# cdglissov/recurrent-flows-msc

Hardware: AMD Instinct MI355X
Metric: frames/sec, RFN SM-MNIST 64x64 train step (fwd+bwd+Adam) (higher is better)
Workload: dtype f32 (forward convolutions fp32-grade: fused scaled-fp16 split f16x3s / three-piece bf16x6 split; gradient convolutions bf16x3 split MFMA; fp32 accumulate everywhere); 1 GPU; RFN SM-MNIST 64x64 canonical (K=10 L=5 Hd=256 h=200 z=56), global_batch=32, seq_len=20, train step; global_batch=32, seq_len=20, parallelism=dp1

## Files before the change

### recurrent-flows-msc_amd/csrc/dgrad_small.hip

```cpp
#include "conv_common.h"
#include <type_traits>

typedef __bf16 bf16x8 __attribute__((ext_vector_type(8)));
typedef __bf16 bf16x4 __attribute__((ext_vector_type(4)));
typedef __bf16 bf16x2 __attribute__((ext_vector_type(2)));

struct DgradSmallParams {
    const float* in;
    long in_ns;
    const unsigned char* wpk;
    float* out1;
    float* out2;
    long out1_ns, out2_ns;
    int Cin, Cout, cout_split, acc1, acc2, CoutP;
    int N, H;
    int CP4;
    int vec;
};

#define DS_MFMA(acc, a, b) acc = __builtin_amdgcn_mfma_f32_32x32x16_bf16(a, b, acc, 0, 0, 0)

template <int CPI>
__device__ __forceinline__ void ds_store_bf16(unsigned char* dst, const __bf16 (&v)[CPI]) {
    if constexpr (CPI == 8) {
        *reinterpret_cast<bf16x8*>(dst) = bf16x8{v[0], v[1], v[2], v[3], v[4], v[5], v[6], v[7]};
    } else if constexpr (CPI == 4) {
        *reinterpret_cast<bf16x4*>(dst) = bf16x4{v[0], v[1], v[2], v[3]};
    } else if constexpr (CPI == 2) {
        *reinterpret_cast<bf16x2*>(dst) = bf16x2{v[0], v[1]};
    } else {
        *reinterpret_cast<__bf16*>(dst) = v[0];
    }
}

template <int W, int MTW, int TPX, int RS>
struct DgradSmallCfg {
    static constexpr int PG = 4 / RS;
    static constexpr int MTT = MTW * RS;
    static constexpr int RPT = 32 / W;
    static constexpr int R = TPX * RPT;
    static constexpr int BPIX = PG * TPX * 32;
    static constexpr bool BAND = BPIX < W * W;
    static constexpr int FPB = BAND ? 1 : BPIX / (W * W);
    static constexpr int PF = BPIX / FPB;
    static constexpr int BR = PF / W;
    static constexpr int IPOSF = (BR + 2) * W, IPOS = FPB * IPOSF;
    static constexpr int IMG_BYTES = 2 * 2 * IPOS * 16;
    static constexpr int WFR = 3 * 2 * MTT;
    static constexpr int WGT_BYTES = WFR * 1024;
    static constexpr int CPI = BPIX / 64;
    static constexpr int NQ = BPIX / 4;
    static constexpr int NLD = CPI + (BAND ? 1 : 0);
    static constexpr int NFI = R + 2 - (RPT - 1);
    static constexpr int ESTR = 36;
    static constexpr int EPI_BYTES = PG * MTT * 32 * ESTR * 4;
    static constexpr int LOOP_BYTES = 2 * IMG_BYTES + 2 * WGT_BYTES;
    static constexpr int LDS_BYTES = LOOP_BYTES > EPI_BYTES ? LOOP_BYTES : EPI_BYTES;
    static_assert(RS == 1 || RS == 2, "row groups");
    static_assert(CPI == 1 || CPI == 2 || CPI == 4 || CPI == 8, "body item shape");
    static_assert(!BAND || W == 32, "bands (halo rows to load) only at W = 32: 2 rows x 16 channels x 8 quads = 256 items");
    static_assert(PF % (TPX * 32) == 0, "a wave's tiles lie in one frame");
    static_assert(LDS_BYTES <= 160 * 1024, "LDS budget");
};

template <int W, int MTW, int TPX, int RS>
__global__ __launch_bounds__(256) void dgrad_small_kernel(const DgradSmallParams p) {
    using C = DgradSmallCfg<W, MTW, TPX, RS>;
    constexpr int PG = C::PG, MTT = C::MTT, RPT = C::RPT, BPIX = C::BPIX, FPB = C::FPB, PF = C::PF, BR = C::BR;
    constexpr int IPOSF = C::IPOSF, IPOS = C::IPOS, IMG_BYTES = C::IMG_BYTES, WFR = C::WFR, WGT_BYTES = C::WGT_BYTES;
    constexpr int CPI = C::CPI, NQ = C::NQ, NLD = C::NLD, NFI = C::NFI, ESTR = C::ESTR;
    constexpr bool BAND = C::BAND;
    constexpr int NJ = (WFR + 3) / 4;
    constexpr unsigned MASKED = 0xFFFFFF00u;
    (void)BPIX; (void)PG;
    extern __shared__ __attribute__((aligned(16))) unsigned char lds[];
    const int tid = threadIdx.x, lane = tid & 63;
    const int wave = __builtin_amdgcn_readfirstlane(tid >> 6);
    const int pg = wave / RS, rs = wave - pg * RS;
    const int l31 = lane & 31, kk = lane >> 5;
    const int HW = p.H * W;
    int n0, rb;
    if (BAND) {
        const int bands = p.H / BR;
        n0 = blockIdx.x / bands;
        rb = (blockIdx.x - n0 * bands) * BR;
    } else {
        n0 = blockIdx.x * FPB;
        rb = 0;
    }
    const int nchunks = p.Cin >> 4;
    const auto rs_in = __builtin_amdgcn_make_buffer_rsrc(const_cast<float*>(p.in), 0,
                                                         (unsigned)((long)p.N * p.in_ns * 4), 0x00020000);

    unsigned b_off, h_off = MASKED;
    int b_dst, h_dst = 0;
    {
        const int cg = tid / NQ, pq = tid - cg * NQ;
        const int f = (pq * 4) / PF, pin = pq * 4 - f * PF;
        const int cl = cg * CPI;
        const bool ok = n0 + f < p.N;
        b_off = ok ? (unsigned)((long)(n0 + f) * p.in_ns * 4) + (unsigned)((cl * HW + rb * W + pin) * 4) : MASKED;
        b_dst = ((cl >> 3) * IPOS + f * IPOSF + W + pin) * 16 + (cl & 7) * 2;
        if (BAND) {
            const int ch = tid >> 4, hr = (tid >> 3) & 1, q = tid & 7;
            const int gy = hr ? rb + BR : rb - 1;
            h_off = (gy >= 0 && gy < p.H) ? (unsigned)((long)n0 * p.in_ns * 4) + (unsigned)((ch * HW + gy * W + 4 * q) * 4)
                                          : MASKED;
            h_dst = ((ch >> 3) * IPOS + (hr ? (BR + 1) * W : 0) + 4 * q) * 16 + (ch & 7) * 2;
        }
    }
    typedef unsigned u32x4_ __attribute__((ext_vector_type(4)));
    auto img_load1 = [&](f32x4 (&raw)[NLD], const int c, const int j) {
        const unsigned base = j < CPI ? b_off : h_off;
        const unsigned off = base == MASKED ? MASKED : base + (unsigned)((c * 16 + (j < CPI ? j : 0)) * HW * 4);
        const u32x4_ v = __builtin_amdgcn_raw_buffer_load_b128(rs_in, off, 0, 0);
        raw[j] = __builtin_bit_cast(f32x4, v);
    };
    auto img_store1 = [&](const f32x4 (&raw)[NLD], const int buf, const int e) {
        unsigned char* img = lds + buf * IMG_BYTES + e * 16;
        __bf16 hi[CPI], lo[CPI];
#pragma unroll
        for (int j = 0; j < CPI; ++j) {
            const float v = raw[j][e];
            hi[j] = (__bf16)v;
            lo[j] = (__bf16)(v - (float)hi[j]);
        }
        ds_store_bf16<CPI>(img + b_dst, hi);
        ds_store_bf16<CPI>(img + b_dst + 2 * IPOS * 16, lo);
        if (BAND) {
            const float v = raw[NLD - 1][e];
            const __bf16 h = (__bf16)v;
            *reinterpret_cast<__bf16*>(img + h_dst) = h;
            *reinterpret_cast<__bf16*>(img + h_dst + 2 * IPOS * 16) = (__bf16)(v - (float)h);
        }
    };
    unsigned w_off[NJ];
#pragma unroll
    for (int j = 0; j < NJ; ++j) {
        const int f = min(wave + 4 * j, WFR - 1);
        const int tp = f / MTT, mt = f - tp * MTT;
        const int dy = tp >> 1, pl = tp & 1;
        const int row = mt * 32 + l31;
        int dx = (row >= p.CP4) + (row >= 2 * p.CP4);
        int co = row - dx * p.CP4;
        if (co >= p.Cout) {
            dx = 0;
            co = p.Cout;
        }
        w_off[j] = (unsigned)((((dy * 3 + dx) * 2 + pl) * 2 + kk) * p.CoutP + co) * 16u;
    }
    const unsigned w_cstride = 36u * (unsigned)p.CoutP * 16u;
    auto wgt_dma = [&](const int c, const int buf) {
        unsigned char* dst0 = lds + 2 * IMG_BYTES + buf * WGT_BYTES;
        const unsigned char* src0 = p.wpk + (size_t)c * w_cstride;
#pragma unroll
        for (int j = 0; j < NJ; ++j) {
            const int f = min(wave + 4 * j, WFR - 1);
            __builtin_amdgcn_global_load_lds((const __attribute__((address_space(1))) void*)(src0 + w_off[j]),
                                             (__attribute__((address_space(3))) void*)(dst0 + f * 1024), 16, 0, 0);
        }
    };
    {
        f32x4* z4 = reinterpret_cast<f32x4*>(lds);
        for (int i = tid; i < 2 * IMG_BYTES / 16; i += 256) z4[i] = f32x4{0.f, 0.f, 0.f, 0.f};
        __syncthreads();
    }

    f32x16 acc[TPX][MTW];
#pragma unroll
    for (int t = 0; t < TPX; ++t)
#pragma unroll
        for (int m = 0; m < MTW; ++m)
#pragma unroll
            for (int r = 0; r < 16; ++r) acc[t][m][r] = 0.f;

    const int wp0 = pg * TPX * 32;
    const int wf = wp0 / PF;
    const int pos0 = wf * IPOSF + (wp0 - wf * PF) + l31;

    f32x4 rawA[NLD], rawB[NLD];
    wgt_dma(0, 0);
#pragma unroll
    for (int j = 0; j < NLD; ++j) img_load1(rawA, 0, j);
#pragma unroll
    for (int j = 0; j < NLD; ++j) img_load1(rawB, 1, j);
#pragma unroll
    for (int e = 0; e < 4; ++e) img_store1(rawA, 0, e);
    asm volatile("s_waitcnt vmcnt(0) lgkmcnt(0)" ::: "memory");
    __syncthreads();

    auto chunk = [&](auto st_, auto ld_, const int c, f32x4 (&rawC)[NLD], f32x4 (&rawN)[NLD]) {
        constexpr bool st = decltype(st_)::value, ld = decltype(ld_)::value;
        const int buf = c & 1;
        const bf16x8* img = reinterpret_cast<const bf16x8*>(lds + buf * IMG_BYTES) + kk * IPOS + pos0;
        const bf16x8* wl = reinterpret_cast<const bf16x8*>(lds + 2 * IMG_BYTES + buf * WGT_BYTES) + rs * MTW * 64 + lane;
        bf16x8 A[3][MTW][2];
#pragma unroll
        for (int dy = 0; dy < 3; ++dy)
#pragma unroll
            for (int m = 0; m < MTW; ++m)
#pragma unroll
                for (int pl = 0; pl < 2; ++pl) A[dy][m][pl] = wl[((dy * 2 + pl) * MTT + m) * 64];
        bf16x8 B[2][2];
        B[0][0] = img[0];
        B[0][1] = img[2 * IPOS];
#pragma unroll
        for (int fi = 0; fi < NFI; ++fi) {
            const int cur = fi & 1;
            if (fi + 1 < NFI) {
                B[cur ^ 1][0] = img[(fi + 1) * W];
                B[cur ^ 1][1] = img[2 * IPOS + (fi + 1) * W];
            }
            __builtin_amdgcn_sched_barrier(0);
#pragma unroll
            for (int combo = 0; combo < 3; ++combo) {
#pragma unroll
                for (int dy = 0; dy < 3; ++dy) {
                    const int ro = (fi - 1) - (dy - 1);
                    if (ro >= 0 && ro <= (TPX - 1) * RPT && ro % RPT == 0) {
#pragma unroll
                        for (int m = 0; m < MTW; ++m) {
                            if (combo == 0) DS_MFMA(acc[ro / RPT][m], A[dy][m][1], B[cur][0]);
                            if (combo == 1) DS_MFMA(acc[ro / RPT][m], A[dy][m][0], B[cur][1]);
                            if (combo == 2) DS_MFMA(acc[ro / RPT][m], A[dy][m][0], B[cur][0]);
                        }
                    }
                }
            }
            constexpr int SS = NFI / 3 > 0 ? NFI / 3 : 1;
#pragma unroll
            for (int k = 0; k < 4; ++k)
                if (st && (k * SS) / 4 == fi) img_store1(rawC, buf ^ 1, k);
            if (st && fi == SS) {
                __builtin_amdgcn_sched_barrier(0);
                wgt_dma(c + 1, buf ^ 1);
                __builtin_amdgcn_sched_barrier(0);
            }
#pragma unroll
            for (int k = 0; k < NLD; ++k)
                if (ld && SS + (k * SS) / NLD == fi) img_load1(rawN, c + 2, k);
            __builtin_amdgcn_sched_barrier(0);
        }
        if (ld) asm volatile("s_waitcnt vmcnt(%0)" ::"n"(NLD) : "memory");
        else asm volatile("s_waitcnt vmcnt(0)" ::: "memory");
        asm volatile("s_waitcnt lgkmcnt(0)" ::: "memory");
        __builtin_amdgcn_s_barrier();
    };
    {
        using T_ = std::integral_constant<bool, true>;
        using F_ = std::integral_constant<bool, false>;
        int c = 0;
        for (; c + 3 < nchunks; c += 2) {
            chunk(T_{}, T_{}, c, rawB, rawA);
            chunk(T_{}, T_{}, c + 1, rawA, rawB);
        }
        chunk(T_{}, F_{}, c, rawB, rawA);
        chunk(F_{}, F_{}, c + 1, rawA, rawB);
    }

    float* E = reinterpret_cast<float*>(lds) + pg * (MTT * 32 * ESTR);
#pragma unroll
    for (int t = 0; t < TPX; ++t) {
        if (t > 0) __syncthreads();
#pragma unroll
        for (int m = 0; m < MTW; ++m)
#pragma unroll
            for (int r = 0; r < 16; ++r)
                E[((rs * MTW + m) * 32 + (r & 3) + 8 * (r >> 2) + 4 * kk) * ESTR + l31] = acc[t][m][r];
        __syncthreads();
        const int wp = wp0 + t * 32;
        const int n = n0 + wf;
        if (n < p.N) {
            const int pix0 = rb * W + (wp - wf * PF);
            for (int idx = rs * 64 + lane; idx < p.Cout * 8; idx += RS * 64) {
                const int co = idx >> 3, q = idx & 7;
                const int x0 = (4 * q) & (W - 1);
                const bool hasL = x0 != 0, hasR = x0 + 4 != W;
                const float* e0 = E + co * ESTR + 4 * q;
                const float* e1 = e0 + p.CP4 * ESTR;
                const float* e2 = e1 + p.CP4 * ESTR;
                const f32x4 a = *reinterpret_cast<const f32x4*>(e0);
                const f32x4 b = *reinterpret_cast<const f32x4*>(e1);
                const f32x4 cc = *reinterpret_cast<const f32x4*>(e2);
                float aL = e0[hasL ? -1 : 0], cR = e2[hasR ? 4 : 0];
                aL = hasL ? aL : 0.f;
                cR = hasR ? cR : 0.f;
                f32x4 o;
                o[0] = aL + b[0] + cc[1];
                o[1] = a[0] + b[1] + cc[2];
                o[2] = a[1] + b[2] + cc[3];
                o[3] = a[2] + b[3] + cR;
                const bool first = co < p.cout_split;
                float* dst = first ? p.out1 + n * p.out1_ns + (long)co * HW + pix0 + 4 * q
                                   : p.out2 + n * p.out2_ns + (long)(co - p.cout_split) * HW + pix0 + 4 * q;
                const bool accm = first ? p.acc1 : p.acc2;
                if (p.vec) {
                    f32x4* d4 = reinterpret_cast<f32x4*>(dst);
                    if (accm) o += *d4;
                    *d4 = o;
                } else {
#pragma unroll
                    for (int e = 0; e < 4; ++e) dst[e] = accm ? o[e] + dst[e] : o[e];
                }
            }
        }
    }
}

template <int W, int MTW, int TPX, int RS>
static int launch_dgrad_small(const DgradSmallParams& p, hipStream_t st) {
    using C = DgradSmallCfg<W, MTW, TPX, RS>;
    constexpr size_t lds = C::LDS_BYTES;
    auto* k = dgrad_small_kernel<W, MTW, TPX, RS>;
    if (lds > 65536) (void)hipFuncSetAttribute((const void*)k, hipFuncAttributeMaxDynamicSharedMemorySize, (int)lds);
    const int blocks = C::BAND ? p.N * (p.H / C::BR) : (p.N + C::FPB - 1) / C::FPB;
    hipLaunchKernelGGL(k, dim3(blocks), dim3(256), lds, st, p);
    return 0;
}

extern "C" int rfn_dgrad_small_supported(int N, int Cin, int Cout, int H, int W) {
    if (N <= 0 || Cin <= 0 || (Cin & 31) || Cout <= 0 || H != W) return 0;
    if ((long)N * Cin * H * W * 4 >= 0xFFFFFF00L) return 0;
    if (W == 32 || W == 16) return Cout <= 64;
    if (W == 8) return Cout <= 96;
    return 0;
}

extern "C" int rfn_conv3x3_smallcout_bf16x3(const float* in, long in_ns, int Cin, const float* wpk, float* out1,
                                            long out1_ns, float* out2, long out2_ns, int Cout, int cout_split, int acc1,
                                            int acc2, int N, int H, int W, rfn_stream_t stream) {
    RFN_CHECK_ARG(in && wpk && out1 && N >= 0, -1);
    RFN_CHECK_ARG(rfn_dgrad_small_supported(N > 0 ? N : 1, Cin, Cout, H, W), -2);
    RFN_CHECK_ARG(cout_split > 0 && cout_split <= Cout && (cout_split == Cout || out2), -3);
    RFN_CHECK_ARG(((uintptr_t)wpk & 15) == 0 && ((uintptr_t)in & 15) == 0 && (in_ns & 3) == 0, -4);
    RFN_CHECK_ARG((long)N * in_ns * 4 < 0xFFFFFF00L && in_ns >= (long)Cin * H * W, -5);
    if (N == 0) return 0;
    DgradSmallParams p;
    p.in = in; p.in_ns = in_ns; p.wpk = reinterpret_cast<const unsigned char*>(wpk);
    p.out1 = out1; p.out2 = out2; p.out1_ns = out1_ns; p.out2_ns = out2_ns;
    p.Cin = Cin; p.Cout = Cout; p.cout_split = cout_split; p.acc1 = acc1; p.acc2 = acc2;
    p.CoutP = ((Cout + 255) / 256) * 256;
    p.N = N; p.H = H;
    p.CP4 = (Cout + 3) & ~3;
    p.vec = ((uintptr_t)out1 & 15) == 0 && (out1_ns & 3) == 0 &&
            (cout_split == Cout || (((uintptr_t)out2 & 15) == 0 && (out2_ns & 3) == 0));
    hipStream_t st = (hipStream_t)stream;
    const int MTR = (3 * p.CP4 + 31) / 32;
    if (W == 32) {
        if (MTR <= 2) launch_dgrad_small<32, 2, 4, 1>(p, st);
        else if (MTR <= 4) launch_dgrad_small<32, 2, 4, 2>(p, st);
        else launch_dgrad_small<32, 3, 4, 2>(p, st);
    } else if (W == 16) {
        if (MTR <= 2) launch_dgrad_small<16, 2, 2, 1>(p, st);
        else if (MTR <= 4) launch_dgrad_small<16, 4, 2, 1>(p, st);
        else launch_dgrad_small<16, 3, 4, 2>(p, st);
    } else {
        if (MTR <= 4) launch_dgrad_small<8, 4, 1, 1>(p, st);
        else if (MTR <= 7 && N >= 512) launch_dgrad_small<8, 7, 1, 1>(p, st);
        else if (MTR <= 8) launch_dgrad_small<8, 4, 1, 2>(p, st);
        else launch_dgrad_small<8, 5, 1, 2>(p, st);
    }
    RFN_LAUNCH_CHECK();
    return 0;
}
```

Before: 12510 frames/s.

## Interleave split-store, weight DMA and MFMA with scheduled groups in dgrad_small chunk loop

Adds a new chunk body for the small dgrad kernel. It issues MFMAs step by step over (dy, tile) and double-buffers the weight fragments in registers. The bf16 hi/lo image split and its LDS writes are spread across those steps. sched_group_barrier enforces an MFMA/DS/VMEM interleave, and the weight DMA is emitted through inline asm with an explicit m0. The aim is to hide LDS traffic, global loads and split arithmetic behind the MFMA pipe. It applies to all configurations except W16/MTW3/TPX4/RS2, and the hand-written asm and strict schedule could raise register pressure or stall.

After: 12540 frames/s, median of 6. About the same (+0.3%).

```diff
diff --git a/recurrent-flows-msc_amd/csrc/dgrad_small.hip b/recurrent-flows-msc_amd/csrc/dgrad_small.hip
--- a/recurrent-flows-msc_amd/csrc/dgrad_small.hip
+++ b/recurrent-flows-msc_amd/csrc/dgrad_small.hip
@@ -56,6 +56,7 @@
     static constexpr int EPI_BYTES = PG * MTT * 32 * ESTR * 4;
     static constexpr int LOOP_BYTES = 2 * IMG_BYTES + 2 * WGT_BYTES;
     static constexpr int LDS_BYTES = LOOP_BYTES > EPI_BYTES ? LOOP_BYTES : EPI_BYTES;
+    static constexpr bool IL = !(W == 16 && MTW == 3 && TPX == 4 && RS == 2);
     static_assert(RS == 1 || RS == 2, "row groups");
     static_assert(CPI == 1 || CPI == 2 || CPI == 4 || CPI == 8, "body item shape");
     static_assert(!BAND || W == 32, "bands (halo rows to load) only at W = 32: 2 rows x 16 channels x 8 quads = 256 items");
@@ -134,6 +135,31 @@
             *reinterpret_cast<__bf16*>(img + h_dst + 2 * IPOS * 16) = (__bf16)(v - (float)h);
         }
     };
+    struct SplitPx {
+        __bf16 hi[CPI], lo[CPI], hh, hl;
+    };
+    auto img_split = [&](const f32x4 (&raw)[NLD], const int e, const int j0, const int j1, SplitPx& sp) {
+#pragma unroll
+        for (int j = j0; j < j1 && j < CPI; ++j) {
+            const float v = raw[j][e];
+            sp.hi[j] = (__bf16)v;
+            sp.lo[j] = (__bf16)(v - (float)sp.hi[j]);
+        }
+        if (BAND && j1 == NLD) {
+            const float v = raw[NLD - 1][e];
+            sp.hh = (__bf16)v;
+            sp.hl = (__bf16)(v - (float)sp.hh);
+        }
+    };
+    auto img_write = [&](const int buf, const int e, const SplitPx& sp) {
+        unsigned char* img = lds + buf * IMG_BYTES + e * 16;
+        ds_store_bf16<CPI>(img + b_dst, sp.hi);
+        ds_store_bf16<CPI>(img + b_dst + 2 * IPOS * 16, sp.lo);
+        if (BAND) {
+            *reinterpret_cast<__bf16*>(img + h_dst) = sp.hh;
+            *reinterpret_cast<__bf16*>(img + h_dst + 2 * IPOS * 16) = sp.hl;
+        }
+    };
     unsigned w_off[NJ];
 #pragma unroll
     for (int j = 0; j < NJ; ++j) {
@@ -160,6 +186,18 @@
                                              (__attribute__((address_space(3))) void*)(dst0 + f * 1024), 16, 0, 0);
         }
     };
+    auto wgt_dma_asm = [&](const int c, const int buf) {
+        const unsigned dst0 = (unsigned)(size_t)(__attribute__((address_space(3))) unsigned char*)(lds + 2 * IMG_BYTES) +
+                              (unsigned)(buf * WGT_BYTES);
+        const unsigned char* src0 = p.wpk + (size_t)c * w_cstride;
+#pragma unroll
+        for (int j = 0; j < NJ; ++j) {
+            const int f = min(wave + 4 * j, WFR - 1);
+            const unsigned m0v = __builtin_amdgcn_readfirstlane(dst0 + (unsigned)f * 1024u);
+            asm volatile("s_mov_b32 m0, %1\n\ts_nop 0\n\tglobal_load_lds_dwordx4 %0, off"
+                         :: "v"(src0 + w_off[j]), "s"(m0v) : "memory");
+        }
+    };
     {
         f32x4* z4 = reinterpret_cast<f32x4*>(lds);
         for (int i = tid; i < 2 * IMG_BYTES / 16; i += 256) z4[i] = f32x4{0.f, 0.f, 0.f, 0.f};
@@ -189,7 +227,83 @@
     asm volatile("s_waitcnt vmcnt(0) lgkmcnt(0)" ::: "memory");
     __syncthreads();
 
-    auto chunk = [&](auto st_, auto ld_, const int c, f32x4 (&rawC)[NLD], f32x4 (&rawN)[NLD]) {
+    auto chunk_il = [&](auto st_, auto ld_, const int c, f32x4 (&rawC)[NLD], f32x4 (&rawN)[NLD]) {
+        constexpr bool st = decltype(st_)::value, ld = decltype(ld_)::value;
+        constexpr int NS = 3 * TPX, NM = 3 * MTW, NA = 2 * MTW;
+        constexpr int NQC = CPI == 8 ? 2 : 1, CQ = CPI / NQC, NU = 4 * NQC, DS = ((NQC - 1) * NS) / NU;
+        constexpr int LSPAN = NS / 2;
+        static_assert(DS + LSPAN < NS, "the image loads lie inside the chunk");
+        const int buf = c & 1;
+        const bf16x8* img = reinterpret_cast<const bf16x8*>(lds + buf * IMG_BYTES) + kk * IPOS + pos0;
+        const bf16x8* wl = reinterpret_cast<const bf16x8*>(lds + 2 * IMG_BYTES + buf * WGT_BYTES) + rs * MTW * 64 + lane;
+        bf16x8 A[2][MTW][2];
+        bf16x8 B[2][2];
+        SplitPx sp[4];
+        B[0][0] = img[0];
+#pragma unroll
+        for (int m = 0; m < MTW; ++m) A[0][m][1] = wl[(1 * MTT + m) * 64];
+        B[0][1] = img[2 * IPOS];
+#pragma unroll
+        for (int m = 0; m < MTW; ++m) A[0][m][0] = wl[m * 64];
+#pragma unroll
+        for (int s = 0; s < NS; ++s) {
+            const int dy = s / TPX, t = s - dy * TPX, cur = s & 1, ab = dy & 1;
+            __builtin_amdgcn_sched_barrier(0);
+            if (s + 1 < NS) {
+                const int fi = ((s + 1) % TPX) * RPT + (s + 1) / TPX;
+                B[cur ^ 1][0] = img[fi * W];
+                B[cur ^ 1][1] = img[2 * IPOS + fi * W];
+            }
+            const bool areads = dy < 2 && t == TPX - 1;
+            if (areads) {
+#pragma unroll
+                for (int r = 0; r < NA; ++r) {
+                    const int pl = r < MTW ? 1 : 0, m = r < MTW ? r : r - MTW;
+                    A[ab ^ 1][m][pl] = wl[(((dy + 1) * 2 + pl) * MTT + m) * 64];
+                }
+            }
+#pragma unroll
+            for (int combo = 0; combo < 3; ++combo) {
+#pragma unroll
+                for (int m = 0; m < MTW; ++m) {
+                    if (combo == 0) DS_MFMA(acc[t][m], A[ab][m][1], B[cur][0]);
+                    if (combo == 1) DS_MFMA(acc[t][m], A[ab][m][0], B[cur][1]);
+                    if (combo == 2) DS_MFMA(acc[t][m], A[ab][m][0], B[cur][0]);
+                }
+            }
+#pragma unroll
+            for (int e = 0; e < 4; ++e)
+                if (st && ((e * NQC + NQC - 1) * NS) / NU + 1 == s) img_write(buf ^ 1, e, sp[e]);
+#pragma unroll
+            for (int u = 0; u < NU; ++u)
+                if (st && (u * NS) / NU == s) {
+                    const int e = u / NQC, q = u - e * NQC;
+                    img_split(rawC, e, q * CQ, q == NQC - 1 ? NLD : (q + 1) * CQ, sp[e]);
+                    if (q == NQC - 1 && s == NS - 1) img_write(buf ^ 1, e, sp[e]);
+                }
+#pragma unroll
+            for (int k = 0; k < NLD; ++k)
+                if (ld && DS + 1 + (k * LSPAN) / NLD == s) img_load1(rawN, c + 2, k);
+#pragma unroll
+            for (int g = 0; g < NM; ++g) {
+                __builtin_amdgcn_sched_group_barrier(0x008, 1, 0);
+                __builtin_amdgcn_sched_group_barrier(0x002, 4, 0);
+                if (g < 2 || (areads && g >= MTW)) __builtin_amdgcn_sched_group_barrier(0x100, 1, 0);
+                __builtin_amdgcn_sched_group_barrier(0x200, 1, 0);
+                __builtin_amdgcn_sched_group_barrier(0x020, 1, 0);
+            }
+            __builtin_amdgcn_sched_barrier(0);
+            if (st && s == DS) {
+                wgt_dma_asm(c + 1, buf ^ 1);
+                __builtin_amdgcn_sched_barrier(0);
+            }
+        }
+        if (ld) asm volatile("s_waitcnt vmcnt(%0)" ::"n"(NLD) : "memory");
+        else asm volatile("s_waitcnt vmcnt(0)" ::: "memory");
+        asm volatile("s_waitcnt lgkmcnt(0)" ::: "memory");
+        __builtin_amdgcn_s_barrier();
+    };
+    auto chunk_fr = [&](auto st_, auto ld_, const int c, f32x4 (&rawC)[NLD], f32x4 (&rawN)[NLD]) {
         constexpr bool st = decltype(st_)::value, ld = decltype(ld_)::value;
         const int buf = c & 1;
         const bf16x8* img = reinterpret_cast<const bf16x8*>(lds + buf * IMG_BYTES) + kk * IPOS + pos0;
@@ -249,6 +363,10 @@
     {
         using T_ = std::integral_constant<bool, true>;
         using F_ = std::integral_constant<bool, false>;
+        auto chunk = [&](auto st_, auto ld_, const int c, f32x4 (&rawC)[NLD], f32x4 (&rawN)[NLD]) {
+            if constexpr (C::IL) chunk_il(st_, ld_, c, rawC, rawN);
+            else chunk_fr(st_, ld_, c, rawC, rawN);
+        };
         int c = 0;
         for (; c + 3 < nchunks; c += 2) {
             chunk(T_{}, T_{}, c, rawB, rawA);
```
